# yuPeiyu98/Diffusion-Amortized-MCMC

Hardware: AMD Instinct MI355X
Metric: Langevin z-steps/sec (B=128, z_dim=128, CIFAR-10) (higher is better)
Workload: dtype f32; 1 GPU; cifar10 train-iteration Langevin block: 30 posterior steps on B=128 + 60 prior steps on 2B=256 split over the ranks (value counts posterior z-steps only); global_batch=128, per_rank_batch=128, per_rank_prior_chains=256, z_dim=128, ngf=128, posterior_steps=30, prior_steps=60, parallelism=dp1 (chains sharded, no collective)

## Files before the change

### diffusion-amortized-mcmc_amd/csrc/gemm.hip

```cpp
#include <algorithm>
#include <atomic>
#include <cstdlib>
#include <type_traits>

#include "gemm.h"

namespace damc {

constexpr int BN = 128;

template <int BK, int MT>
struct TileCfg {
  static constexpr int BM = 64 * MT;
  static constexpr int LDA = (BK == 16) ? BM + 2 : BM + 1;
  static constexpr int LDB = BN;
  static constexpr int AQ = BK / 4;
  static constexpr int AROWS_V = BM * BK / 1024;
  static constexpr int AROWS_S = BM * BK / 256;
  static constexpr int BROWS_V = BK / 8;
  static constexpr int BROWS_S = BK / 2;
};

template <int OM>
__device__ __forceinline__ long gemm_row_offset(const GemmArgs& p, int m, int py, int px) {
// ... 867 lines not shown
    const long v = e ? atol(e) : 0;
    return (v > 0 && v < 2147483647L) ? v : 2147483647L;
  }();
  const long per = (lim / 4 - 1) / img;
  if (per < 1) return DAMC_ERR_UNSUPPORTED;
  const long cimg = (om == O_PHASE) ? (long)a.Hout * a.Wout * a.ldc : hwq * a.ldc;
  for (long b0 = 0; b0 < nimg; b0 += per) {
    const long nb = std::min(per, nimg - b0);
    GemmArgs c = a;
    c.A = a.A + b0 * img;
    c.C = a.C + b0 * cimg;
    if (a.mask) c.mask = a.mask + b0 * cimg;
    c.M = (int)(nb * hwq);
    const char* esk = getenv("DAMC_KM_SKINNY");
    const char* ekr = getenv("DAMC_KM_SKINNY_ROWS");
    const int km_rows = ekr ? atoi(ekr) : 64;
    if (epi == EPI_STORE && om == O_DENSE && c.M <= km_rows && c.Hin == 1 && c.Win == 1 && c.Hq == 1 && c.Wq == 1 &&
        c.kw == 1 && c.Cg == c.K && !(esk && esk[0] == '0')) {
      const dim3 g((unsigned)zdim, (unsigned)((c.N + 127) / 128), (unsigned)((c.M + 31) / 32));
      hipLaunchKernelGGL(km_skinny_kernel, g, dim3(256), 0, s, c);
      continue;
    }
#define DAMC_KM(E_, O_)                \
  if (epi == E_ && om == O_) {         \
    launch_km_t<E_, O_>(c, zdim, s);   \
    continue;                          \
  }
    DAMC_KM(EPI_BIAS_ACT, O_PHASE)
    DAMC_KM(EPI_MASK, O_DENSE)
    DAMC_KM(EPI_BIAS_ACT, O_DENSE)
    DAMC_KM(EPI_STORE, O_DENSE)
#undef DAMC_KM
    return DAMC_ERR_UNSUPPORTED;
  }
  return (int)hipGetLastError();
}

constexpr int X3_BM = 256, X3_BN = 128, X3_BK = 32, X3_ROWB = 192;
__device__ __forceinline__ int x3_swz(int row) { return (row >> 1) & 3; }
constexpr int X3_F32A = 2097152, X3A_ROWB = 128;
constexpr int X3_NARROW = 4194304;
constexpr int X3_TAPSHARE = 16777216;
__device__ __forceinline__ int f32a_swz(int r) { return ((r >> 1) & 7) ^ ((((r >> 2) ^ (r >> 3)) & 1) << 1); }
__device__ __forceinline__ int ts_swz(int r) { return ((r >> 1) & 1) | (((r >> 2) & 1) << 2); }
static_assert(X3_NEGK % 32 == 0 && (X3_NEGK & (X3_NEGK - 1)) == 0, "sign blocks are whole K tiles, a power of two");
constexpr int X3_CHUNKS = 12;
typedef __bf16 bf16x8 __attribute__((ext_vector_type(8)));
typedef unsigned int u32x4 __attribute__((ext_vector_type(4)));
template <int N>
using x3_ic = std::integral_constant<int, N>;

constexpr int X3_BASE = 261, X3_RASTER = 16, X3_WIDE = 524288, X3_KREG = 1048576;
constexpr int X3_BITS = X3_BASE | X3_RASTER | X3_WIDE | X3_KREG | X3_F32A | X3_NARROW | X3_TAPSHARE;
__device__ __forceinline__ void split3_octet(const float (&v)[8], bf16x8& h, bf16x8& m, bf16x8& l) {
#pragma unroll
  for (int e = 0; e < 8; ++e) {
    const __bf16 b0 = (__bf16)v[e];
    const float r1 = sub_rn(v[e], (float)b0);
    const __bf16 b1 = (__bf16)r1;
    const float r2 = sub_rn(r1, (float)b1);
    h[e] = b0;
    m[e] = b1;
    l[e] = (__bf16)r2;
  }
}

template <int NT>
__device__ __forceinline__ void proj16(const float* tile, int ts, int r0, int C, const float* w, int ldw,
                                       f32x4 (&acc)[NT]) {
  const int lane = threadIdx.x & 63, m = lane & 15, q = lane >> 4;
#pragma unroll
  for (int t = 0; t < NT; ++t) acc[t] = f32x4{0.f, 0.f, 0.f, 0.f};
  for (int g = 0; g < C / 16; ++g) {
    const f32x4 a = *reinterpret_cast<const f32x4*>(tile + (r0 + m) * ts + 16 * g + 4 * q);
#pragma unroll
    for (int t = 0; t < NT; ++t) {
      const f32x4 b = *reinterpret_cast<const f32x4*>(w + (long)(16 * t + m) * ldw + 16 * g + 4 * q);
#pragma unroll
      for (int e = 0; e < 4; ++e) acc[t] = __builtin_amdgcn_mfma_f32_16x16x4f32(a[e], b[e], acc[t], 0, 0, 0);
    }
  }
}

template <int NT>
__global__ __launch_bounds__(512) void proj_rows_kernel(const float* __restrict__ h, long npix, int C,
                                                        const float* __restrict__ w, int ldw, float* __restrict__ P,
                                                        long pstride) {
  constexpr int TS = 256 + 4;
  __shared__ __attribute__((aligned(16))) float tile[128 * TS];
  const int tid = threadIdx.x, wave = tid >> 6, lane = tid & 63;
  const long p0 = (long)blockIdx.x * 128;
  const int c4 = C / 4;
  for (int i = tid; i < 128 * c4; i += 512) {
    const int r = i / c4, c = (i - r * c4) * 4;
    const long pix = p0 + r;
    *reinterpret_cast<f32x4*>(tile + r * TS + c) =
        pix < npix ? *reinterpret_cast<const f32x4*>(h + pix * C + c) : f32x4{0.f, 0.f, 0.f, 0.f};
  }
  __syncthreads();
  const int m = lane & 15, q = lane >> 4;
  for (int c0 = 0; c0 < C; c0 += PROJ_CHUNK) {
    f32x4 acc[NT];
    proj16<NT>(tile + c0, TS, wave * 16, min(PROJ_CHUNK, C - c0), w + c0, ldw, acc);
    float* Pc = P + (c0 / PROJ_CHUNK) * pstride;
#pragma unroll
    for (int t = 0; t < NT; ++t)
#pragma unroll
      for (int r = 0; r < 4; ++r) {
        const long pix = p0 + wave * 16 + 4 * q + r;
        if (pix < npix) Pc[pix * (16 * NT) + 16 * t + m] = acc[t][r];
      }
  }
}

int launch_proj_rows(const float* h, long npix, int C, const float* w, int ldw, int np, float* P, long pstride,
                     hipStream_t s) {
  if (C <= 0 || C > 256 || C % 16 || (np != 32 && np != 64) || npix <= 0) return DAMC_ERR_ARG;
  if (C > PROJ_CHUNK && pstride < npix * np) return DAMC_ERR_ARG;
  const dim3 grid((unsigned)((npix + 127) / 128));
  if (np == 32)
    hipLaunchKernelGGL(proj_rows_kernel<2>, grid, dim3(512), 0, s, h, npix, C, w, ldw, P, pstride);
  else
    hipLaunchKernelGGL(proj_rows_kernel<4>, grid, dim3(512), 0, s, h, npix, C, w, ldw, P, pstride);
  return (int)hipGetLastError();
}

template <int EPI, int OM, int V = X3_BASE>
__global__ __launch_bounds__(512, (V & X3_NARROW) ? 2 : 1) void gemm_x3_kernel(GemmArgs p) {
  static_assert((V & X3_BASE) == X3_BASE && !(V & ~X3_BITS), "V: X3_BASE and the named variant bits only");
  constexpr bool WIDE = (V & X3_WIDE) != 0;
  constexpr bool NARROW = (V & X3_NARROW) != 0;
  static_assert(!NARROW || !(V & (X3_RASTER | X3_WIDE | X3_KREG | X3_F32A)), "NARROW: the default limb path, unsplit");
  constexpr int BM = WIDE ? 128 : NARROW ? 64 : X3_BM, BN = WIDE ? 256 : X3_BN;
  constexpr bool F32A = (V & X3_F32A) != 0;
  static_assert(!F32A || (OM != O_WGRAD && !WIDE), "F32A: 256 x 128 tiles, not the weight gradient");
  constexpr int AROWB = F32A ? X3A_ROWB : X3_ROWB, ESZ = F32A ? 4 : 6;
  constexpr int AJ = (BM * (F32A ? 8 : X3_CHUNKS) + 511) / 512, BJ = BN * X3_CHUNKS / 512;
  constexpr int BUFB = BM * AROWB + BN * X3_ROWB;
  constexpr int TS_NT = OM == O_PHASE ? 4 : 16;
  constexpr int TS_STG = BM * X3_ROWB, TS_B = TS_STG + BM * X3A_ROWB, TS_ZERO = TS_B + 2 * BN * X3_ROWB;
  constexpr int TS_TOFF = TS_ZERO + 4 * X3_ROWB, TS_END = TS_TOFF + TS_NT * BM * 4;
  constexpr int SMEMB =
      ((V & X3_TAPSHARE) && TS_END > 2 * (BM + BN) * X3_ROWB) ? TS_END : 2 * (BM + BN) * X3_ROWB;
  static_assert(SMEMB <= 160 * 1024 && TS_ZERO % 256 == 0, "the LDS of a CU; zero rows on the images' bank phase");
  const int FLOG = __builtin_ctz((unsigned)p.negk >> 5), FLUSH = 1 << FLOG;
  __shared__ __attribute__((aligned(16))) unsigned char smem[SMEMB];
  const int tid = threadIdx.x;
  const int lane = tid & 63;
  const int wave = tid >> 6;
  const int wm = (WIDE || NARROW) ? wave >> 2 : wave >> 1, wn = (WIDE || NARROW) ? wave & 3 : wave & 1;
  unsigned long long clk_t0 = 0, clk_r0 = 0;
  if (p.clk && tid == 0) {
    clk_t0 = __builtin_amdgcn_s_memtime();
    clk_r0 = __builtin_amdgcn_s_memrealtime();
  }
  constexpr bool RASTER = (V & X3_RASTER) != 0 && OM != O_WGRAD;
  const int wgid = xcd_remap(blockIdx.x, gridDim.x);
  const int ntn = (p.N + BN - 1) / BN;
  int tm, tn, z;
  if constexpr (RASTER) {
    const int nph = OM == O_PHASE ? 4 : 1;
    const int ntm = (p.M + BM - 1) / BM;
    int pr;
    supertile(wgid, ntm, ntn * nph, tm, pr);
    tn = pr / nph;
    z = pr - tn * nph;
// ... 209 lines not shown
      if (kt + 1 < nk) dma_n(kbeg + (kt + 1) * X3_BK, (kt + 1) & 1);
      bf16x8 fa[2][3], fb[2][3];
#pragma unroll
      for (int t = 0; t < 2; ++t)
#pragma unroll
        for (int l = 0; l < 3; ++l) {
          fa[t][l] = *reinterpret_cast<const bf16x8*>(base + afn + t * 16 * X3_ROWB + oct16 + l * 16);
          fb[t][l] = *reinterpret_cast<const bf16x8*>(base + bfn + t * 16 * X3_ROWB + oct16 + l * 16);
        }
#pragma unroll
      for (int i = 0; i < 2; ++i)
#pragma unroll
        for (int j = 0; j < 2; ++j) {
          f32x4 c = acc16[i][j];
          c = __builtin_amdgcn_mfma_f32_16x16x32_bf16(fa[i][2], fb[j][0], c, 0, 0, 0);
          c = __builtin_amdgcn_mfma_f32_16x16x32_bf16(fa[i][1], fb[j][1], c, 0, 0, 0);
          c = __builtin_amdgcn_mfma_f32_16x16x32_bf16(fa[i][0], fb[j][2], c, 0, 0, 0);
          c = __builtin_amdgcn_mfma_f32_16x16x32_bf16(fa[i][1], fb[j][0], c, 0, 0, 0);
          c = __builtin_amdgcn_mfma_f32_16x16x32_bf16(fa[i][0], fb[j][1], c, 0, 0, 0);
          acc16[i][j] = __builtin_amdgcn_mfma_f32_16x16x32_bf16(fa[i][0], fb[j][0], c, 0, 0, 0);
        }
      __syncthreads();
      if (((kt + 1) & (FLUSH - 1)) == 0) {
        const float sg = (p.b_negblk && (((kt + kt0) >> FLOG) & 1)) ? -1.f : 1.f;
#pragma unroll
        for (int i = 0; i < 2; ++i)
#pragma unroll
          for (int j = 0; j < 2; ++j) {
#pragma unroll
            for (int r = 0; r < 4; ++r) tot16[i][j][r] = __builtin_fmaf(sg, acc16[i][j][r], tot16[i][j][r]);
            acc16[i][j] = f32x4{0.f, 0.f, 0.f, 0.f};
          }
      }
    }
  } else if constexpr (F32A) {
    auto dma_a = [&](int buf) {
      unsigned char* dst = smem + buf * BUFB + wbase;
#pragma unroll
      for (int j = 0; j < AJ; ++j)
        __builtin_amdgcn_raw_ptr_buffer_load_lds(rsA, (lds_t)(dst + 512 * 16 * j), 16, (int)aoff[j], ci0 * ESZ, 0, 0);
      next_ktile();
    };
    constexpr int BOFF = TSHARE ? TS_B : BM * X3A_ROWB, BBUF = TSHARE ? BN * X3_ROWB : BUFB;
    const int wbase_s = TSHARE ? __builtin_amdgcn_readfirstlane(wbase) : 0;
    auto dma_b = [&](int k0, int buf) {
      unsigned char* dst = smem + buf * BBUF + BOFF + (TSHARE ? wbase_s : wbase);
#pragma unroll
      for (int j = 0; j < BJ; ++j)
        __builtin_amdgcn_raw_ptr_buffer_load_lds(rsB, (lds_t)(dst + 512 * 16 * j), 16, (int)boff[j], k0 * 6, 0, 0);
    };
    const int fs = f32a_swz(lrow);
    const int ca0 = ((2 * loct) ^ fs) * 16, ca1 = ((2 * loct + 1) ^ fs) * 16;
    const int arow = (wave * 32 + lrow) * X3A_ROWB, brow = BOFF + lrow * X3_ROWB + oct16;
    auto rd_a = [&](const unsigned char* buf, f32x4 (&av)[2][2]) {
#pragma unroll
      for (int a = 0; a < 2; ++a) {
        av[a][0] = *reinterpret_cast<const f32x4*>(buf + arow + a * 16 * X3A_ROWB + ca0);
        av[a][1] = *reinterpret_cast<const f32x4*>(buf + arow + a * 16 * X3A_ROWB + ca1);
      }
    };
    auto split2 = [&](const f32x4 (&av)[2][2], bf16x8 (&f)[2][3], int a, int e) {
#pragma unroll
      for (int d = 0; d < 2; ++d) {
        const float v = av[a][(e + d) >> 2][(e + d) & 3];
        const __bf16 b0 = (__bf16)v;
        const float r1 = sub_rn(v, (float)b0);
        const __bf16 b1 = (__bf16)r1;
        const float r2 = sub_rn(r1, (float)b1);
        f[a][0][e + d] = b0;
        f[a][1][e + d] = b1;
        f[a][2][e + d] = (__bf16)r2;
      }
    };
    auto rd_split = [&](const unsigned char* buf, bf16x8 (&f)[2][3]) {
      f32x4 av[2][2];
      rd_a(buf, av);
#pragma unroll
      for (int a = 0; a < 2; ++a)
#pragma unroll
        for (int e = 0; e < 8; e += 2) split2(av, f, a, e);
    };
    unsigned ts_ibase = 0;
    int ts_nv = 0, ts_pstr = 0;
    if constexpr (TSHARE) {
      constexpr int NT = TS_NT;
      const int r0 = tid >> 3, mi = m0 + r0;
      const unsigned b = mi / hwq, r = mi - b * hwq, qy = r / p.Wq, qx = r - qy * p.Wq;
      ts_ibase = ((b * p.Hin + qy * p.stride) * Win + qx * p.stride) * Cg * 4 + ((tid & 7) ^ ts_swz(r0)) * 16;
      ts_nv = min(4, max(0, (p.M - mi + 63) >> 6));
      ts_pstr = ((64 % hwq == 0) ? (64 / hwq) * p.Hin * Win : (64 / p.Wq) * p.stride * Win) * Cg * 4;
      for (int id = tid; id < NT * BM; id += 512) {
        const int row = id & (BM - 1), pos = id >> 8, m = m0 + row;
        int ky, kx, dlt;
        if constexpr (OM == O_PHASE) {
          ky = pos >> 1;
          kx = pos & 1;
          dlt = (ky - pad_y) * p.Wq + kx - pad_x;
        } else {
          const int c = pos >> 2, jj = pos & 3, tp = x3_walk_tap(pos);
          ky = tp >> 2;
          kx = tp & 3;
          dlt = ((jj >> 1) - 1 + (c >> 1)) * p.Wq + (jj & 1) - 1 + (c & 1);
        }
        const int bb = m / hwq, rr = m - bb * hwq, y = rr / p.Wq, x = rr - y * p.Wq;
        const int R = row + dlt;
        const bool live = m < p.M && (unsigned)(y * p.stride - pad_y + ky) < (unsigned)p.Hin &&
                          (unsigned)(x * p.stride - pad_x + kx) < (unsigned)Win && (unsigned)R < (unsigned)BM;
        reinterpret_cast<int*>(smem + TS_TOFF)[id] = (live ? R * X3_ROWB : TS_ZERO + (R & 3) * X3_ROWB) + x3_swz(R) * 16;
      }
      if (tid < 4 * X3_ROWB / 4) reinterpret_cast<float*>(smem + TS_ZERO)[tid] = 0.f;
    }
    auto dma_img = [&](int G, int j) {
      const int gg = (kt0 >> 2) + G;
      int sl = gg, coff = 0;
      if constexpr (OM == O_DENSE) {
        const int c = gg & 3;
        sl = gg >> 2;
        coff = ((1 - (c >> 1)) * Win + (1 - (c & 1))) * Cg * 4;
      }
      unsigned char* dst = smem + TS_STG + wbase_s + 512 * 16 * j;
      const int vo = j < ts_nv ? (int)(ts_ibase + (unsigned)(j * ts_pstr)) : (int)KM_OOB;
      __builtin_amdgcn_raw_ptr_buffer_load_lds(rsA, (lds_t)dst, 16, vo, sl * (X3_BK * 4) + coff, 0, 0);
    };
    const int ts_tb = TS_TOFF + (wm * 64 + lrow) * 4;
    auto ts_addr = [&](int ktn, int (&o)[4]) {
      const int ta = ts_tb + ((kt0 + ktn) & (TS_NT - 1)) * (BM * 4);
#pragma unroll
      for (int i = 0; i < 4; ++i) o[i] = *reinterpret_cast<const int*>(smem + ta + i * 64) ^ (loct << 4);
    };
    const int cv_rd = TS_STG + (wave * 32 + lrow) * X3A_ROWB + ((2 * loct) ^ ts_swz(lrow)) * 16;
    auto rd_stg = [&](f32x4 (&av)[2][2], int a) {
      av[a][0] = *reinterpret_cast<const f32x4*>(smem + cv_rd + a * 16 * X3A_ROWB);
      av[a][1] = *reinterpret_cast<const f32x4*>(smem + (cv_rd ^ 16) + a * 16 * X3A_ROWB);
    };
    const int cv_wr = (wave * 32 + lrow) * X3_ROWB + (loct ^ sw) * 16;
    auto wr_limb = [&](const bf16x8 (&f)[2][3], int a) {
#pragma unroll
      for (int l = 0; l < 3; ++l) *reinterpret_cast<bf16x8*>(smem + cv_wr + a * 16 * X3_ROWB + l * 64) = f[a][l];
    };
    bf16x8 fx[2][3], fy[2][3], fb[2][3];
    constexpr int SG_MFMA = 0x8, SG_VALU = 0x2, SG_DS_RD = 0x100, SG_DS_WR = 0x200;
    auto mfma6 = [&](const bf16x8 (&fc)[2][3], int t) {
      const int sl = t & 1;
#pragma unroll
      for (int a = 0; a < 2; ++a) {
        f32x4 c = acc16[2 * a + (t >> 2)][t & 3];
        c = __builtin_amdgcn_mfma_f32_16x16x32_bf16(fc[a][2], fb[sl][0], c, 0, 0, 0);
        c = __builtin_amdgcn_mfma_f32_16x16x32_bf16(fc[a][1], fb[sl][1], c, 0, 0, 0);
        c = __builtin_amdgcn_mfma_f32_16x16x32_bf16(fc[a][0], fb[sl][2], c, 0, 0, 0);
        c = __builtin_amdgcn_mfma_f32_16x16x32_bf16(fc[a][1], fb[sl][0], c, 0, 0, 0);
        c = __builtin_amdgcn_mfma_f32_16x16x32_bf16(fc[a][0], fb[sl][1], c, 0, 0, 0);
        acc16[2 * a + (t >> 2)][t & 3] = __builtin_amdgcn_mfma_f32_16x16x32_bf16(fc[a][0], fb[sl][0], c, 0, 0, 0);
      }
    };
    auto flush_blk = [&](int kt) {
      if constexpr (KREG) {
        const float sg = (p.b_negblk && (((kt + kt0) >> FLOG) & 1)) ? -1.f : 1.f;
        const int ntile = ((p.M + BM - 1) / BM) * ((p.N + BN - 1) / BN);
        const __amdgpu_buffer_rsrc_t rsl = __builtin_amdgcn_make_buffer_rsrc(
            (void*)(p.kslab + ((long)zph * p.ksplit + zsl * p.kbpw) * ntile * (BM * BN)), (short)0,
            p.kbpw * ntile * (BM * BN) * 4, 0x00020000);
        const int soff = ((kt >> FLOG) * ntile + tm * ntn + tn) * (BM * BN * 4);
        if constexpr (TSHARE) {
          const int voff = (wave * 1024 + lane) * 16;
#pragma unroll
          for (int i = 0; i < 4; ++i)
#pragma unroll
            for (int j = 0; j < 4; ++j) {
              acc16[i][j] *= sg;
              if (m0 + wm * 64 + i * 16 < p.M)
                __builtin_amdgcn_raw_buffer_store_b128(__builtin_bit_cast(u32x4, acc16[i][j]), rsl,
                                                       voff + soff + (i * 4 + j) * 1024, 0, 0);
              acc16[i][j] = f32x4{0.f, 0.f, 0.f, 0.f};
            }
          return;
        }
        const int voff = ((wave >> 1) * 2 * 1024 + ((wave & 1) * 2) * 4 * 64 + lane) * 16;
#pragma unroll
        for (int i = 0; i < 4; ++i)
#pragma unroll
          for (int j = 0; j < 4; ++j) {
            const int a = i >> 1, wnp = i & 1;
            acc16[i][j] *= sg;
            if (m0 + wave * 32 + a * 16 < p.M) {
              __builtin_amdgcn_raw_buffer_store_b128(__builtin_bit_cast(u32x4, acc16[i][j]), rsl,
                                                     voff + soff + (wnp * 1024 + (a * 4 + j) * 64) * 16, 0, 0);
            }
            acc16[i][j] = f32x4{0.f, 0.f, 0.f, 0.f};
          }
      } else {
        flush16(kt);
      }
    };
    if constexpr (TSHARE) {
      int oa[4], ob[4];
      if (nk > 0) {
#pragma unroll
        for (int j = 0; j < 4; ++j) dma_img(0, j);
        dma_b(kbeg, 0);
      }
      __syncthreads();
      {
        f32x4 av0[2][2];
#pragma unroll
        for (int a = 0; a < 2; ++a) {
          rd_stg(av0, a);
#pragma unroll
          for (int e = 0; e < 8; e += 2) split2(av0, fx, a, e);
          wr_limb(fx, a);
        }
      }
      ts_addr(0, oa);
      __syncthreads();
      bf16x8 pa[3];
      auto tile = [&](int kt, auto PH_, int (&oc)[4], int (&on)[4]) {
        constexpr int PH = decltype(PH_)::value;
        constexpr bool PFI = PH > 0, PFO = PH < 3;
        const unsigned char* base = smem + (PH & 1) * BBUF;
        if constexpr (PH < 3) {
          if (kt + 1 < nk) dma_b(kbeg + (kt + 1) * X3_BK, (PH + 1) & 1);
          const int G = (kt >> 2) + 1;
          if (4 * G < nk) {
            if constexpr (PH == 0) dma_img(G, 0);
            dma_img(G, PH + 1);
          }
        }
        bf16x8 fa[4][3], fq[2][3], fl[2][3];
        f32x4 av[2][2];
        auto rd_a = [&](int i) {
#pragma unroll
          for (int l = 0; l < 3; ++l) fa[i][l] = *reinterpret_cast<const bf16x8*>(smem + oc[i] + l * 64);
        };
        auto rd_b = [&](int j) {
#pragma unroll
          for (int l = 0; l < 3; ++l)
            fq[j & 1][l] = *reinterpret_cast<const bf16x8*>(base + brow + (wn * 64 + j * 16) * X3_ROWB + l * 16);
        };
        auto mf = [&](int i, int j) {
          const int sl = j & 1;
          f32x4 c = acc16[i][j];
          c = __builtin_amdgcn_mfma_f32_16x16x32_bf16(fa[i][2], fq[sl][0], c, 0, 0, 0);
          c = __builtin_amdgcn_mfma_f32_16x16x32_bf16(fa[i][1], fq[sl][1], c, 0, 0, 0);
          c = __builtin_amdgcn_mfma_f32_16x16x32_bf16(fa[i][0], fq[sl][2], c, 0, 0, 0);
          c = __builtin_amdgcn_mfma_f32_16x16x32_bf16(fa[i][1], fq[sl][0], c, 0, 0, 0);
          c = __builtin_amdgcn_mfma_f32_16x16x32_bf16(fa[i][0], fq[sl][1], c, 0, 0, 0);
          acc16[i][j] = __builtin_amdgcn_mfma_f32_16x16x32_bf16(fa[i][0], fq[sl][0], c, 0, 0, 0);
        };
        auto pin = [&](auto N_, auto V_) {
#pragma unroll
          for (int m = 0; m < decltype(N_)::value; ++m) {
            __builtin_amdgcn_sched_group_barrier(SG_MFMA, 1, 0);
            if constexpr (decltype(V_)::value > 0) __builtin_amdgcn_sched_group_barrier(SG_VALU, 1, 0);
            if constexpr (decltype(V_)::value > 1) __builtin_amdgcn_sched_group_barrier(SG_VALU, 1, 0);
          }
        };
        constexpr x3_ic<0> V0{};
        constexpr x3_ic<PH == 3 ? 2 : 0> V2{};
        if constexpr (PFI) {
#pragma unroll
          for (int l = 0; l < 3; ++l) fa[0][l] = pa[l];
        } else {
          rd_a(0);
        }
        rd_b(0);
        rd_a(1);
        mf(0, 0);
        rd_a(2);
        mf(1, 0);
        rd_a(3);
        mf(2, 0);
        rd_b(1);
        ts_addr(kt + 1, on);
        if constexpr (PH == 3) rd_stg(av, 0);
        mf(3, 0);
        __builtin_amdgcn_sched_group_barrier(SG_DS_RD, PFI ? 3 : 6, 0);
        pin(x3_ic<1>{}, V0);
        __builtin_amdgcn_sched_group_barrier(SG_DS_RD, 3, 0);
        pin(x3_ic<5>{}, V0);
        __builtin_amdgcn_sched_group_barrier(SG_DS_RD, 3, 0);
        pin(x3_ic<6>{}, V0);
        __builtin_amdgcn_sched_group_barrier(SG_DS_RD, 3, 0);
        pin(x3_ic<6>{}, V0);
        __builtin_amdgcn_sched_group_barrier(SG_DS_RD, PH == 3 ? 3 + 2 + 2 : 3 + 2, 0);
// ... 136 lines not shown
        rd_a(0);
        rd_b(0);
        rd_b(1);
        mf(0, 0);
        rd_b(2);
        mf(0, 1);
        rd_b(3);
        mf(0, 2);
        rd_a(1);
        mf(0, 3);
        rd_a(2);
#pragma unroll
        for (int j = 0; j < 4; ++j) mf(1, j);
        rd_a(3);
#pragma unroll
        for (int i = 2; i < 4; ++i)
#pragma unroll
          for (int j = 0; j < 4; ++j) mf(i, j);
        __builtin_amdgcn_sched_group_barrier(SG_DS_RD, 9, 0);
        __builtin_amdgcn_sched_group_barrier(SG_MFMA, 6, 0);
        __builtin_amdgcn_sched_group_barrier(SG_DS_RD, 3, 0);
        __builtin_amdgcn_sched_group_barrier(SG_MFMA, 6, 0);
        __builtin_amdgcn_sched_group_barrier(SG_DS_RD, 3, 0);
        __builtin_amdgcn_sched_group_barrier(SG_MFMA, 6, 0);
        __builtin_amdgcn_sched_group_barrier(SG_DS_RD, 3, 0);
        __builtin_amdgcn_sched_group_barrier(SG_MFMA, 6, 0);
        __builtin_amdgcn_sched_group_barrier(SG_DS_RD, 3, 0);
        __builtin_amdgcn_sched_group_barrier(SG_MFMA, 24, 0);
        __builtin_amdgcn_sched_group_barrier(SG_DS_RD, 3, 0);
        __builtin_amdgcn_sched_group_barrier(SG_MFMA, 48, 0);
        __syncthreads();
        if (KREG) {
          if (((kt + 1) & (FLUSH - 1)) != 0) continue;
          const float sg = (p.b_negblk && (((kt + kt0) >> FLOG) & 1)) ? -1.f : 1.f;
          const int ntile = ((p.M + BM - 1) / BM) * ((p.N + BN - 1) / BN);
          const __amdgpu_buffer_rsrc_t rsl = __builtin_amdgcn_make_buffer_rsrc(
              (void*)(p.kslab + ((long)zph * p.ksplit + zsl * p.kbpw) * ntile * (BM * BN)), (short)0,
              p.kbpw * ntile * (BM * BN) * 4, 0x00020000);
          const int soff = ((kt >> FLOG) * ntile + tm * ntn + tn) * (BM * BN * 4);
          const int voff = (wave * 1024 + lane) * 16;
          const bool live = m0 + wm * 64 < p.M;
#pragma unroll
          for (int i = 0; i < 4; ++i)
#pragma unroll
            for (int j = 0; j < 4; ++j) {
              acc16[i][j] *= sg;
              if (live)
                __builtin_amdgcn_raw_buffer_store_b128(__builtin_bit_cast(u32x4, acc16[i][j]), rsl, voff,
                                                       soff + (i * 4 + j) * 1024, 0);
              acc16[i][j] = f32x4{0.f, 0.f, 0.f, 0.f};
            }
        } else if (((kt + 1) & (FLUSH - 1)) == 0) {
          flush16(kt);
        }
      }
    };
    kloop();
  }
  if (p.clk && tid == 0) {
    const unsigned long long t1 = __builtin_amdgcn_s_memtime(), r1 = __builtin_amdgcn_s_memrealtime();
    unsigned long long* c = p.clk + 4 * ((blockIdx.z * gridDim.x + blockIdx.x) % (unsigned)p.clk_n);
    c[0] = clk_t0;
    c[1] = clk_r0;
    c[2] = t1;
    c[3] = r1;
  }
  if (KREG) return;
  {
    const float sg = (p.b_negblk && nk > 0 && (((nk - 1 + kt0) >> FLOG) & 1)) ? -1.f : 1.f;
    constexpr int MI = NARROW ? 2 : 4;
#pragma unroll
    for (int i = 0; i < MI; ++i)
#pragma unroll
      for (int j = 0; j < MI; ++j)
#pragma unroll
        for (int r = 0; r < 4; ++r) acc16[i][j][r] = __builtin_fmaf(sg, acc16[i][j][r], tot16[i][j][r]);
  }
  constexpr int TS = BN + 4;
  static_assert(BM * TS * 4 + BM * 8 <= 2 * (BM + BN) * X3_ROWB, "epilogue tile exceeds the LDS");
  float* tile = reinterpret_cast<float*>(smem);
  long* rowtab = reinterpret_cast<long*>(smem + BM * TS * 4);
  float* Cz = p.C;
  if ((OM == O_DENSE || OM == O_WGRAD) && Cz) Cz += (long)(KSPLIT ? zph : z) * p.c_zstride;
  auto octet = [&](int row, int oct) {
    const int n = n0 + oct * 8;
    const long rowoff = rowtab[row];
    if (rowoff < 0 || n >= p.N) return;
    const long idx = rowoff + n;
    const f32x4 t0 = *reinterpret_cast<const f32x4*>(tile + row * TS + oct * 8);
    const f32x4 t1 = *reinterpret_cast<const f32x4*>(tile + row * TS + oct * 8 + 4);
    float v[8] = {t0.x, t0.y, t0.z, t0.w, t1.x, t1.y, t1.z, t1.w};
    if (EPI == EPI_BIAS_ACT) {
      if (p.bias) {
        const int nb = p.bias_mod < p.N ? n % p.bias_mod : n;
        const f32x4 b0 = *reinterpret_cast<const f32x4*>(p.bias + nb);
        const f32x4 b1 = *reinterpret_cast<const f32x4*>(p.bias + nb + 4);
        const float bb[8] = {b0.x, b0.y, b0.z, b0.w, b1.x, b1.y, b1.z, b1.w};
#pragma unroll
        for (int e = 0; e < 8; ++e) v[e] += bb[e];
      }
#pragma unroll
      for (int e = 0; e < 8; ++e) v[e] = act_apply(v[e], p.act, p.slope);
    } else if (EPI == EPI_MASK) {
      if (p.mask_sgn) {
        const unsigned bits = p.mask_sgn[idx >> 3];
#pragma unroll
        for (int e = 0; e < 8; ++e) v[e] *= ((bits >> e) & 1u) ? 1.f : p.mask_slope;
      } else {
        const f32x4 k0 = *reinterpret_cast<const f32x4*>(p.mask + idx);
        const f32x4 k1 = *reinterpret_cast<const f32x4*>(p.mask + idx + 4);
        const float kk[8] = {k0.x, k0.y, k0.z, k0.w, k1.x, k1.y, k1.z, k1.w};
#pragma unroll
        for (int e = 0; e < 8; ++e) v[e] *= act_grad_from_out(kk[e], p.mask_act, p.mask_slope);
      }
    }
    if (p.sgn) {
      unsigned bits = 0;
#pragma unroll
      for (int e = 0; e < 8; ++e) bits |= (v[e] > 0.f ? 1u : 0u) << e;
      p.sgn[idx >> 3] = (unsigned char)bits;
    }
    if (Cz && !p.proj_nostore) {
      *reinterpret_cast<f32x4*>(Cz + idx) = f32x4{v[0], v[1], v[2], v[3]};
      *reinterpret_cast<f32x4*>(Cz + idx + 4) = f32x4{v[4], v[5], v[6], v[7]};
    }
    if (p.C3) {
      bf16x8 h, m, l;
      split3_octet(v, h, m, l);
      bf16x8* o = reinterpret_cast<bf16x8*>(p.C3 + 3 * idx);
      o[0] = h;
      o[1] = m;
      o[2] = l;
    }
    if ((OM == O_PHASE && EPI == EPI_BIAS_ACT && (WIDE || F32A) && p.proj_out) ||
        (OM == O_DENSE && EPI == EPI_BIAS_ACT && !WIDE && !NARROW && p.in_part)) {
      *reinterpret_cast<f32x4*>(tile + row * TS + oct * 8) = f32x4{v[0], v[1], v[2], v[3]};
      *reinterpret_cast<f32x4*>(tile + row * TS + oct * 8 + 4) = f32x4{v[4], v[5], v[6], v[7]};
    }
  };
  auto epilogue = [&]() {
#pragma unroll 2
    for (int it = 0; it < BM * BN / 8 / 512; ++it) {
      const int id = tid + 512 * it;
      octet(id / (BN / 8), id % (BN / 8));
    }
    if constexpr (OM == O_PHASE && EPI == EPI_BIAS_ACT && (WIDE || F32A)) {
      if (p.proj_out) {
        __syncthreads();
        const int m = lane & 15, q = lane >> 4;
        auto store = [&](auto NT_) {
          constexpr int NT = decltype(NT_)::value;
          constexpr int RG = F32A ? 2 : 1;
          int ptid = tid;
          if constexpr (TSHARE) asm volatile("" : "+v"(ptid));
#pragma unroll
          for (int g = 0; g < RG; ++g) {
            const int r0 = F32A ? (TSHARE ? ptid >> 6 : wave) * 32 + g * 16 : wave * 16;
            __builtin_amdgcn_sched_barrier(0);
            for (int c0 = 0; c0 < (F32A ? BN : p.N); c0 += PROJ_CHUNK) {
              const int cc = F32A ? n0 : c0;
              if (cc >= p.N) break;
              f32x4 acc[NT];
              proj16<NT>(tile + c0, TS, r0, min(PROJ_CHUNK, p.N - cc), p.proj_w + cc, p.proj_ldw, acc);
              float* Pc = p.proj_out + (cc / PROJ_CHUNK) * p.proj_pstride;
#pragma unroll
              for (int t = 0; t < NT; ++t)
#pragma unroll
                for (int r = 0; r < 4; ++r) {
                  const long ro = rowtab[r0 + 4 * q + r];
                  if (ro >= 0) Pc[(ro / p.ldc) * (16 * NT) + 16 * t + m] = acc[t][r];
                }
            }
          }
        };
        if (p.proj_np == 32)
          store(std::integral_constant<int, 2>{});
        else
          store(std::integral_constant<int, 4>{});
      }
    }
  };
  if (tid < BM) rowtab[tid] = (m0 + tid < p.M) ? gemm_row_offset<OM>(p, m0 + tid, py, px) : -1L;
  if (F32A && !TSHARE) {
#pragma unroll
    for (int i = 0; i < 4; ++i)
#pragma unroll
      for (int j = 0; j < 4; ++j)
#pragma unroll
        for (int r = 0; r < 4; ++r)
          tile[(wave * 32 + (i >> 1) * 16 + 4 * (lane >> 4) + r) * TS + ((i & 1) * 4 + j) * 16 + (lane & 15)] =
              acc16[i][j][r];
  } else if (NARROW) {
#pragma unroll
    for (int i = 0; i < 2; ++i)
#pragma unroll
      for (int j = 0; j < 2; ++j)
#pragma unroll
        for (int r = 0; r < 4; ++r)
          tile[(wm * 32 + i * 16 + 4 * (lane >> 4) + r) * TS + wn * 32 + j * 16 + (lane & 15)] = acc16[i][j][r];
  } else {
#pragma unroll
    for (int i = 0; i < 4; ++i)
#pragma unroll
      for (int j = 0; j < 4; ++j)
#pragma unroll
        for (int r = 0; r < 4; ++r)
          tile[(wm * 64 + i * 16 + 4 * (lane >> 4) + r) * TS + wn * 64 + j * 16 + (lane & 15)] = acc16[i][j][r];
  }
  __syncthreads();
  if (KSPLIT) {
    float* sl = p.kslab + ((long)zph * p.ksplit + zsl) * p.M * p.N;
#pragma unroll 2
    for (int it = 0; it < BM * BN / 8 / 512; ++it) {
      const int id = tid + 512 * it, row = id / (BN / 8), oct = id % (BN / 8);
      const int m = m0 + row, n = n0 + oct * 8;
      if (m >= p.M || n >= p.N) continue;
      float* d = sl + (long)m * p.N + n;
      *reinterpret_cast<f32x4*>(d) = *reinterpret_cast<const f32x4*>(tile + row * TS + oct * 8);
      *reinterpret_cast<f32x4*>(d + 4) = *reinterpret_cast<const f32x4*>(tile + row * TS + oct * 8 + 4);
    }
    return;
  }
  epilogue();
  if constexpr (OM == O_DENSE && EPI == EPI_BIAS_ACT && !WIDE && !NARROW && BM == 256 && BN == 128) {
    static_assert(BM * TS * 4 + BM * 8 + 1024 * 4 <= 2 * (BM + BN) * X3_ROWB, "statistics scratch exceeds the LDS");
    if (p.in_part && !KSPLIT) {
      __syncthreads();
      float* red = reinterpret_cast<float*>(smem + BM * TS * 4 + BM * 8);
      float st[3];
      strip256_stats(tile, TS, tid, n0 + (tid & 127) < p.N, red, st);
      if (tid < 128 && n0 + tid < p.N) {
        const int b = m0 / p.in_hw, sp = (m0 - b * p.in_hw) >> 8;
        float* o = p.in_part + (((long)b * p.N + n0 + tid) * p.in_S + sp) * 3;
        o[0] = st[0];
        o[1] = st[1];
        o[2] = st[2];
      }
    }
  }
}

template <int EPI, int OM>
__device__ __forceinline__ void x3_octet_epilogue(const GemmArgs& p, int m, int n, int py, int px, float (&v)[8]);
template <int EPI>
__device__ __forceinline__ void x3_octet_epilogue_at(const GemmArgs& p, long idx, int n, float (&v)[8]);

template <int EPI, int OM>
__global__ __launch_bounds__(256) void x3_ksplit_reduce_tile_kernel(GemmArgs p, int zdim) {
  __shared__ float red[4][16][17];
  const int lane = threadIdx.x & 63, w = threadIdx.x >> 6;
  const long blk = (long)blockIdx.x * 4 + w;
  const int ntm = (p.M + X3_BM - 1) / X3_BM, ntn = (p.N + X3_BN - 1) / X3_BN;
  const long ntile = (long)ntm * ntn;
  const int ij = (int)(blk & 15), wave = (int)((blk >> 4) & 7);
  const long tl = blk >> 7;
  const int tile = (int)(tl % ntile), ph = (int)(tl / ntile);
  const int tm = tile / ntn, tn = tile - tm * ntn;
  const int m0 = tm * X3_BM + (wave >> 1) * 64 + (ij >> 2) * 16, n0 = tn * X3_BN + (wave & 1) * 64 + (ij & 3) * 16;
  const bool live = ph < zdim && m0 < p.M && n0 < p.N;
  f32x4 v = {0.f, 0.f, 0.f, 0.f};
  if (live) {
    const long sstride = ntile * (X3_BM * X3_BN / 4);
    const f32x4* src = reinterpret_cast<const f32x4*>(p.kslab) + (long)ph * p.ksplit * sstride +
                       (((long)tile * 8 + wave) * 16 + ij) * 64 + lane;
    int sl = 0;
    for (; sl + 4 <= p.ksplit; sl += 4) {
      const f32x4 t0 = src[(long)sl * sstride], t1 = src[(long)(sl + 1) * sstride];
      const f32x4 t2 = src[(long)(sl + 2) * sstride], t3 = src[(long)(sl + 3) * sstride];
      v += t0;
      v += t1;
      v += t2;
      v += t3;
    }
    for (; sl < p.ksplit; ++sl) v += src[(long)sl * sstride];
  }
#pragma unroll
  for (int r = 0; r < 4; ++r) red[w][4 * (lane >> 4) + r][lane & 15] = v[r];
  __syncthreads();
  if (!live || lane >= 32) return;
  const int row = lane >> 1, oc = (lane & 1) * 8, m = m0 + row, n = n0 + oc;
  if (m >= p.M || n >= p.N) return;
  float o[8];
#pragma unroll
  for (int c = 0; c < 8; ++c) o[c] = red[w][row][oc + c];
  const int py = OM == O_PHASE ? ph >> 1 : 0, px = OM == O_PHASE ? ph & 1 : 0;
  x3_octet_epilogue<EPI, OM>(p, m, n, py, px, o);
}

template <int NT>
__global__ __launch_bounds__(256) void x3_ksplit_reduce_proj_kernel(GemmArgs p, int zdim) {
  constexpr int TS = X3_BN + 4, RW = 64;
  __shared__ __attribute__((aligned(16))) float tile[RW * TS];
  __shared__ long rowtab[RW];
  __shared__ int rowpix[RW];
  const int tid = threadIdx.x, lane = tid & 63, w = tid >> 6;
  const int ntm = (p.M + X3_BM - 1) / X3_BM, ntn = (p.N + X3_BN - 1) / X3_BN;
  const long ntile = (long)ntm * ntn;
  const int qtr = blockIdx.x & 3;
  const long tl = blockIdx.x >> 2;
  const int tile_i = (int)(tl % ntile), ph = (int)(tl / ntile);
  if (ph >= zdim) return;
  const int tm = tile_i / ntn, tn = tile_i - tm * ntn;
  const int py = ph >> 1, px = ph & 1;
  const int r16 = qtr * RW + 16 * w;
  const int wm = r16 >> 6, ti = (r16 & 63) >> 4;
  const long sstride = ntile * (X3_BM * X3_BN / 4);
// ... 1016 lines not shown
```

Before: 61230 z-steps/s.

## Specialize tap-shared GEMM epilogue with register-resident projection weights and shift-based indexing

For the tap-sharing GEMM path, adds a dedicated epilogue that hoists the bias load per thread, builds row tables once, and fuses the downstream projection using weights prefetched into registers before the tile stores. The tap-offset table construction now uses shifts and masks instead of divisions (assuming power-of-two spatial dims), is unrolled, and is moved after the DMA issue so it overlaps with loads. The intent is to cut integer division cost, redundant bias and weight global loads, and epilogue latency. It adds register pressure from the weight buffer and relies on power-of-two hwq and Wq.

```diff
diff --git a/diffusion-amortized-mcmc_amd/csrc/gemm.hip b/diffusion-amortized-mcmc_amd/csrc/gemm.hip
--- a/diffusion-amortized-mcmc_amd/csrc/gemm.hip
+++ b/diffusion-amortized-mcmc_amd/csrc/gemm.hip
@@ -973,6 +973,33 @@
   }
 }
 
+template <int NT, int G0 = 0, int G1 = PROJ_CHUNK / 16>
+__device__ __forceinline__ void proj16_load_w(const float* w, int ldw, int cw, f32x4 (&wb)[PROJ_CHUNK / 16][NT]) {
+  const int lane = threadIdx.x & 63, m = lane & 15, q = lane >> 4;
+#pragma unroll
+  for (int g = G0; g < G1; ++g)
+#pragma unroll
+    for (int t = 0; t < NT; ++t)
+      wb[g][t] = 16 * g < cw ? *reinterpret_cast<const f32x4*>(w + (long)(16 * t + m) * ldw + 16 * g + 4 * q)
+                             : f32x4{0.f, 0.f, 0.f, 0.f};
+}
+template <int NT>
+__device__ __forceinline__ void proj16_w(const float* tile, int ts, int r0, int cw, const f32x4 (&wb)[PROJ_CHUNK / 16][NT],
+                                         f32x4 (&acc)[NT]) {
+  const int lane = threadIdx.x & 63, m = lane & 15, q = lane >> 4;
+#pragma unroll
+  for (int t = 0; t < NT; ++t) acc[t] = f32x4{0.f, 0.f, 0.f, 0.f};
+#pragma unroll
+  for (int g = 0; g < PROJ_CHUNK / 16; ++g) {
+    if (16 * g >= cw) break;
+    const f32x4 a = *reinterpret_cast<const f32x4*>(tile + (r0 + m) * ts + 16 * g + 4 * q);
+#pragma unroll
+    for (int t = 0; t < NT; ++t)
+#pragma unroll
+      for (int e = 0; e < 4; ++e) acc[t] = __builtin_amdgcn_mfma_f32_16x16x4f32(a[e], wb[g][t][e], acc[t], 0, 0, 0);
+  }
+}
+
 template <int NT>
 __global__ __launch_bounds__(512) void proj_rows_kernel(const float* __restrict__ h, long npix, int C,
                                                         const float* __restrict__ w, int ldw, float* __restrict__ P,
@@ -1348,15 +1375,22 @@
     };
     unsigned ts_ibase = 0;
     int ts_nv = 0, ts_pstr = 0;
+    [[maybe_unused]] const int ts_lhw = TSHARE ? __builtin_ctz((unsigned)hwq) : 0,
+                               ts_lwq = TSHARE ? __builtin_ctz((unsigned)p.Wq) : 0;
     if constexpr (TSHARE) {
-      constexpr int NT = TS_NT;
       const int r0 = tid >> 3, mi = m0 + r0;
-      const unsigned b = mi / hwq, r = mi - b * hwq, qy = r / p.Wq, qx = r - qy * p.Wq;
+      const unsigned b = (unsigned)mi >> ts_lhw, r = mi & (hwq - 1), qy = r >> ts_lwq, qx = r & (p.Wq - 1);
       ts_ibase = ((b * p.Hin + qy * p.stride) * Win + qx * p.stride) * Cg * 4 + ((tid & 7) ^ ts_swz(r0)) * 16;
       ts_nv = min(4, max(0, (p.M - mi + 63) >> 6));
-      ts_pstr = ((64 % hwq == 0) ? (64 / hwq) * p.Hin * Win : (64 / p.Wq) * p.stride * Win) * Cg * 4;
-      for (int id = tid; id < NT * BM; id += 512) {
-        const int row = id & (BM - 1), pos = id >> 8, m = m0 + row;
+      ts_pstr = ((64 % hwq == 0) ? (64 >> ts_lhw) * p.Hin * Win : (64 >> ts_lwq) * p.stride * Win) * Cg * 4;
+    }
+    auto ts_table = [&]() {
+      const int row = tid & (BM - 1), m = m0 + row;
+      const int rr = m & (hwq - 1), y = rr >> ts_lwq, x = rr & (p.Wq - 1);
+      const int iy = y * p.stride - pad_y, ix = x * p.stride - pad_x;
+#pragma unroll
+      for (int k = 0; k < TS_NT / 2; ++k) {
+        const int pos = (tid >> 8) + 2 * k;
         int ky, kx, dlt;
         if constexpr (OM == O_PHASE) {
           ky = pos >> 1;
@@ -1368,14 +1402,14 @@
           kx = tp & 3;
           dlt = ((jj >> 1) - 1 + (c >> 1)) * p.Wq + (jj & 1) - 1 + (c & 1);
         }
-        const int bb = m / hwq, rr = m - bb * hwq, y = rr / p.Wq, x = rr - y * p.Wq;
         const int R = row + dlt;
-        const bool live = m < p.M && (unsigned)(y * p.stride - pad_y + ky) < (unsigned)p.Hin &&
-                          (unsigned)(x * p.stride - pad_x + kx) < (unsigned)Win && (unsigned)R < (unsigned)BM;
-        reinterpret_cast<int*>(smem + TS_TOFF)[id] = (live ? R * X3_ROWB : TS_ZERO + (R & 3) * X3_ROWB) + x3_swz(R) * 16;
+        const bool live = m < p.M && (unsigned)(iy + ky) < (unsigned)p.Hin && (unsigned)(ix + kx) < (unsigned)Win &&
+                          (unsigned)R < (unsigned)BM;
+        reinterpret_cast<int*>(smem + TS_TOFF)[tid + 512 * k] =
+            (live ? R * X3_ROWB : TS_ZERO + (R & 3) * X3_ROWB) + x3_swz(R) * 16;
       }
       if (tid < 4 * X3_ROWB / 4) reinterpret_cast<float*>(smem + TS_ZERO)[tid] = 0.f;
-    }
+    };
     auto dma_img = [&](int G, int j) {
       const int gg = (kt0 >> 2) + G;
       int sl = gg, coff = 0;
@@ -1465,6 +1499,7 @@
         for (int j = 0; j < 4; ++j) dma_img(0, j);
         dma_b(kbeg, 0);
       }
+      ts_table();
       __syncthreads();
       {
         f32x4 av0[2][2];
@@ -1767,6 +1802,143 @@
   long* rowtab = reinterpret_cast<long*>(smem + BM * TS * 4);
   float* Cz = p.C;
   if ((OM == O_DENSE || OM == O_WGRAD) && Cz) Cz += (long)(KSPLIT ? zph : z) * p.c_zstride;
+  if constexpr (TSHARE) {
+    if (!KSPLIT) {
+      static_assert(BM * TS * 4 + BM * 8 + BM * 4 <= SMEMB, "epilogue tile and row tables exceed the LDS");
+      int* rowpix = reinterpret_cast<int*>(smem + BM * TS * 4 + BM * 8);
+      auto ts_epilogue = [&](auto NT_) {
+        constexpr int NT = decltype(NT_)::value;
+        constexpr bool PROJ = NT > 0;
+        f32x4 wb[PROJ_CHUNK / 16][PROJ ? NT : 1];
+        const int cw = min(PROJ_CHUNK, p.N - n0);
+        constexpr int GW = NT <= 2 ? PROJ_CHUNK / 16 : PROJ_CHUNK / 32;
+        if constexpr (PROJ) proj16_load_w<NT, 0, GW>(p.proj_w + n0, p.proj_ldw, cw, wb);
+        if (tid < BM) {
+          const int m = m0 + tid;
+          long pix = -1;
+          if (m < p.M) {
+            if constexpr (OM == O_PHASE) {
+              const int lhw = __builtin_ctz((unsigned)hwq), lwq = __builtin_ctz((unsigned)p.Wq);
+              const int b = m >> lhw, rr = m & (hwq - 1), qy = rr >> lwq, qx = rr & (p.Wq - 1);
+              pix = ((long)b * p.Hout + 2 * qy + py) * p.Wout + 2 * qx + px;
+            } else {
+              pix = m;
+            }
+          }
+          rowtab[tid] = pix < 0 ? -1L : pix * p.ldc;
+          if constexpr (PROJ) rowpix[tid] = (int)pix;
+        }
+#pragma unroll
+        for (int i = 0; i < 4; ++i)
+#pragma unroll
+          for (int j = 0; j < 4; ++j)
+#pragma unroll
+            for (int r = 0; r < 4; ++r)
+              tile[(wm * 64 + i * 16 + 4 * (lane >> 4) + r) * TS + wn * 64 + j * 16 + (lane & 15)] = acc16[i][j][r];
+        __syncthreads();
+        auto octet8 = [&](int row, int oct, long idx, const float (&bb)[8], unsigned mbits) -> unsigned {
+          const f32x4 t0 = *reinterpret_cast<const f32x4*>(tile + row * TS + oct * 8);
+          const f32x4 t1 = *reinterpret_cast<const f32x4*>(tile + row * TS + oct * 8 + 4);
+          float v[8] = {t0.x, t0.y, t0.z, t0.w, t1.x, t1.y, t1.z, t1.w};
+          if (EPI == EPI_BIAS_ACT) {
+            if (p.bias) {
+#pragma unroll
+              for (int e = 0; e < 8; ++e) v[e] += bb[e];
+            }
+#pragma unroll
+            for (int e = 0; e < 8; ++e) v[e] = act_apply(v[e], p.act, p.slope);
+          } else if (EPI == EPI_MASK) {
+            if (p.mask_sgn) {
+#pragma unroll
+              for (int e = 0; e < 8; ++e) v[e] *= ((mbits >> e) & 1u) ? 1.f : p.mask_slope;
+            } else {
+              const f32x4 k0 = *reinterpret_cast<const f32x4*>(p.mask + idx);
+              const f32x4 k1 = *reinterpret_cast<const f32x4*>(p.mask + idx + 4);
+              const float kk[8] = {k0.x, k0.y, k0.z, k0.w, k1.x, k1.y, k1.z, k1.w};
+#pragma unroll
+              for (int e = 0; e < 8; ++e) v[e] *= act_grad_from_out(kk[e], p.mask_act, p.mask_slope);
+            }
+          }
+          unsigned bits = 0;
+#pragma unroll
+          for (int e = 0; e < 8; ++e) bits |= (v[e] > 0.f ? 1u : 0u) << e;
+          if (Cz && !p.proj_nostore) {
+            *reinterpret_cast<f32x4*>(Cz + idx) = f32x4{v[0], v[1], v[2], v[3]};
+            *reinterpret_cast<f32x4*>(Cz + idx + 4) = f32x4{v[4], v[5], v[6], v[7]};
+          }
+          if (p.C3) {
+            bf16x8 h, m, l;
+            split3_octet(v, h, m, l);
+            bf16x8* o = reinterpret_cast<bf16x8*>(p.C3 + 3 * idx);
+            o[0] = h;
+            o[1] = m;
+            o[2] = l;
+          }
+          if constexpr (PROJ) {
+            *reinterpret_cast<f32x4*>(tile + row * TS + oct * 8) = f32x4{v[0], v[1], v[2], v[3]};
+            *reinterpret_cast<f32x4*>(tile + row * TS + oct * 8 + 4) = f32x4{v[4], v[5], v[6], v[7]};
+          }
+          return bits;
+        };
+        {
+          float bb[8] = {};
+          if (EPI == EPI_BIAS_ACT && p.bias && n0 + (tid & 15) * 8 < p.N) {
+            const int n = n0 + (tid & 15) * 8;
+            const int nb = p.bias_mod < p.N ? n % p.bias_mod : n;
+            const f32x4 b0 = *reinterpret_cast<const f32x4*>(p.bias + nb);
+            const f32x4 b1 = *reinterpret_cast<const f32x4*>(p.bias + nb + 4);
+            bb[0] = b0.x, bb[1] = b0.y, bb[2] = b0.z, bb[3] = b0.w;
+            bb[4] = b1.x, bb[5] = b1.y, bb[6] = b1.z, bb[7] = b1.w;
+          }
+#pragma unroll 2
+          for (int it = 0; it < BM * BN / 8 / 512; ++it) {
+            const int id = tid + 512 * it, row = id / (BN / 8), oct = id % (BN / 8);
+            const int n = n0 + oct * 8;
+            const long rowoff = rowtab[row];
+            if (rowoff < 0 || n >= p.N) continue;
+            const long idx = rowoff + n;
+            const unsigned mb = (EPI == EPI_MASK && p.mask_sgn) ? p.mask_sgn[idx >> 3] : 0u;
+            const unsigned sg = octet8(row, oct, idx, bb, mb);
+            if (p.sgn) p.sgn[idx >> 3] = (unsigned char)sg;
+          }
+        }
+        if constexpr (PROJ) {
+          if constexpr (GW < PROJ_CHUNK / 16)
+            proj16_load_w<NT, GW, PROJ_CHUNK / 16>(p.proj_w + n0, p.proj_ldw, cw, wb);
+          __syncthreads();
+          const int m = lane & 15, q = lane >> 4;
+          int ptid = tid;
+          asm volatile("" : "+v"(ptid));
+          float* Pc = p.proj_out + (n0 / PROJ_CHUNK) * p.proj_pstride;
+#pragma unroll
+          for (int g = 0; g < 2; ++g) {
+            const int r0 = (ptid >> 6) * 32 + g * 16;
+            __builtin_amdgcn_sched_barrier(0);
+            f32x4 acc[PROJ ? NT : 1];
+            proj16_w<PROJ ? NT : 1>(tile, TS, r0, cw, wb, acc);
+#pragma unroll
+            for (int r = 0; r < 4; ++r) {
+              const int pix = rowpix[r0 + 4 * q + r];
+#pragma unroll
+              for (int t = 0; t < NT; ++t)
+                if (pix >= 0) Pc[(long)pix * (16 * NT) + 16 * t + m] = acc[t][r];
+            }
+          }
+        }
+      };
+      if constexpr (OM == O_PHASE && EPI == EPI_BIAS_ACT) {
+        if (p.proj_out) {
+          if (p.proj_np == 32)
+            ts_epilogue(std::integral_constant<int, 2>{});
+          else
+            ts_epilogue(std::integral_constant<int, 4>{});
+          return;
+        }
+      }
+      ts_epilogue(std::integral_constant<int, 0>{});
+      return;
+    }
+  }
   auto octet = [&](int row, int oct) {
     const int n = n0 + oct * 8;
     const long rowoff = rowtab[row];
@@ -1906,7 +2078,7 @@
     }
     return;
   }
-  epilogue();
+  if constexpr (!TSHARE) epilogue();
   if constexpr (OM == O_DENSE && EPI == EPI_BIAS_ACT && !WIDE && !NARROW && BM == 256 && BN == 128) {
     static_assert(BM * TS * 4 + BM * 8 + 1024 * 4 <= 2 * (BM + BN) * X3_ROWB, "statistics scratch exceeds the LDS");
     if (p.in_part && !KSPLIT) {
```

After: 61990 z-steps/s, median of 6. 1.01x the previous value.
